# zhu-xlab/PFST

Measured on AMD Instinct MI355X. Metric: PFST train-step images/s on 1024² IRRG tiles, higher is better.
Workload: dtype f32 (f16x3 split MFMA: two scaled fp16 pieces per operand, three products, fp32 accumulate); 1 GPU; pfst_pots_irrg2vaih_irrg_deeplabv3plus_r50-d8; global_batch=8, per_gpu_batch=8, tile=1024x1024x3, num_classes=6, parallelism=dp1, weights=seeded random init, conv_math=f16x3

## Files before the change

### include/pfst_hip.h

```cpp
#ifndef PFST_HIP_H
#define PFST_HIP_H
#ifdef __cplusplus
extern "C" {
#endif

typedef void* pfst_stream_t;

int pfst_abi_version(void);
const char* pfst_last_error(void);
int pfst_set_deterministic(int on);
int pfst_get_deterministic(void);

int pfst_fill_f32(float* p, long long n, float value, pfst_stream_t stream);
int pfst_axpy_f32(float* y, const float* x, float alpha, long long n, pfst_stream_t stream);
int pfst_i64_to_u8(const long long* src, unsigned char* dst, long long n, pfst_stream_t stream);
int pfst_u8_to_i64(const unsigned char* src, long long* dst, long long n, pfst_stream_t stream);

typedef struct pfst_bnb_fuse {
  const float* x;
  long long x_bs;
  const float* y;
  long long y_bs;
  const float* coef;
  float* partials;
// ... 14 lines not shown
int pfst_conv_pack_weight_split(const float* w, void* wk6_fprop, void* wk6_dgrad, int Cout, int Cin, int T, pfst_stream_t stream);
int pfst_conv_igemm_split(const float* in, long long in_bs, const void* wk6, const float* bias, float* out, long long out_bs,
                          int N, int C, int Hi, int Wi, int M, int Ho, int Wo, int ksize, int stride, int dil, int pad,
                          int mode, int accumulate, float* stats, const pfst_bnb_fuse_t* bnb, pfst_stream_t stream);
int pfst_conv_wgrad_split(const float* x, long long x_bs, const float* dy, long long dy_bs, float* dw,
                          int N, int Cin, int Hi, int Wi, int Cout, int Ho, int Wo, int ksize, int stride, int dil, int pad,
                          pfst_stream_t stream);
int pfst_conv_wgrad(const float* x, long long x_bs, const float* dy, long long dy_bs, float* dw,
                    int N, int Cin, int Hi, int Wi, int Cout, int Ho, int Wo, int ksize, int stride, int dil, int pad,
                    pfst_stream_t stream);
int pfst_conv_wgrad_set_lds_pad(int bytes);
int pfst_bias_grad(const float* dy, long long dy_bs, float* db, int N, int C, int HW, pfst_stream_t stream);

int pfst_wino_tiles(int H, int W, int dil, int m);
int pfst_wino_pack_weight(const float* w, float* U_fprop, float* U_dgrad, int Cout, int Cin, int m, pfst_stream_t stream);
int pfst_wino_input(const float* x, long long x_bs, float* V, int N, int C, int H, int W, int dil, int m, float* v_amax,
                    const float* pack_x_amax, const float* bnl, pfst_stream_t stream);
int pfst_wino_gemm(const float* V, const float* U, float* Mbuf, int N, int K, int M, int T, int m, pfst_stream_t stream);
int pfst_wino_output(const float* Mbuf, float* y, long long y_bs, int N, int Cout, int H, int W, int dil, int accumulate,
                     float* stats, int stats_minmax, const float* bnb_x, long long bnb_x_bs, const float* bnb_coef, int bnb_relu, int m,
                     pfst_stream_t stream);
int pfst_wino_stats_slots(int H, int W, int dil, int m);
int pfst_wino_dy(const float* dy, long long dy_bs, float* dM, int N, int Cout, int H, int W, int dil, int m, float* dm_amax,
                 const float* pack_dy_amax, pfst_stream_t stream);
int pfst_wino_wgrad(const float* V, const float* dM, float* dU, float* dw, int N, int Cin, int Cout, int T, int m,
                    int split, const float* v_amax, const float* dm_amax, int packed, pfst_stream_t stream);
int pfst_wino_filter_plain(const float* w, float* P_fprop, float* P_dgrad, int Cout, int Cin, int m, pfst_stream_t stream);
int pfst_wino_pack_weight_split(const float* plain_f, const float* plain_d, void* U6_fprop, void* U6_dgrad, int Cout, int Cin,
                                int m, pfst_stream_t stream);
int pfst_wino_gemm_split(const float* V, const void* U6, float* Mbuf, int N, int K, int M, int T, int m, pfst_stream_t stream);

int pfst_absmax(const float* x, long long n, int planes, long long plane_stride, int slot_stride, float* slots, pfst_stream_t stream);
int pfst_conv_pack_weight_f16x2(const float* w, void* wk4_fprop, void* wk4_dgrad, int Cout, int Cin, int T, int sets,
                                const float* amax, pfst_stream_t stream);
typedef struct pfst_weight_job {
  const float* src;
  void* dst_f;
  void* dst_d;
  float* amax_f;
  float* amax_d;
  int Cout, Cin, T, sets, m, first_block;
} pfst_weight_job_t;
int pfst_weight_job_blocks(const pfst_weight_job_t* job, int pack);
int pfst_weight_prep_batched(const pfst_weight_job_t* jobs_host, const pfst_weight_job_t* jobs_dev, int njobs, pfst_stream_t stream);
int pfst_conv_pack_weight_f16x2_batched(const pfst_weight_job_t* jobs_host, const pfst_weight_job_t* jobs_dev, int njobs,
                                        pfst_stream_t stream);
int pfst_conv_igemm_f16x3(const float* in, long long in_bs, const void* wk4, const float* w_amax, const float* in_amax,
                          const float* bias, float* out, long long out_bs, int N, int C, int Hi, int Wi, int M, int Ho, int Wo,
                          int ksize, int stride, int dil, int pad, int mode, int accumulate, float* stats, const pfst_bnb_fuse_t* bnb,
                          const float* gate_dy, long long gate_dy_bs, const unsigned long long* gate_mask, int stats_minmax,
                          const float* bnl, pfst_stream_t stream);
int pfst_f16x3_set_slots(int slots);
int pfst_f16x3_chain_grid(long long total_tiles, int chainable);
int pfst_f16x3_split_probe(const float* x, long long n, const float* amax, unsigned* pieces_loop, unsigned* pieces_loop4,
                           unsigned* pieces_plain, pfst_stream_t stream);
int pfst_wino_gemm_f16x3(const float* V, const void* U4, const float* u_amax, const float* v_amax, float* Mbuf, int N, int K,
                         int M, int T, int m, int v_packed, pfst_stream_t stream);
int pfst_conv_wgrad_f16x3(const float* x, long long x_bs, const float* dy, long long dy_bs, float* dw, int N, int Cin, int Cout,
                          int HW, const float* x_amax, const float* dy_amax, const float* bnl, pfst_stream_t stream);
int pfst_conv_wgrad_f16x3_q(const float* x, long long x_bs, const float* dy, long long dy_bs, float* dw, int N, int Cin, int H, int W,
                            int Cout, int ksize, int dil, const float* x_amax, const float* dy_amax, pfst_stream_t stream);

int pfst_dwconv3x3(const float* x, long long x_bs, const float* w, float* y, long long y_bs,
                   int N, int C, int H, int W, int dil, int flip, int accumulate, float* stats, int stats_minmax,
                   const float* bn_on_load_coef, pfst_stream_t stream);
int pfst_dwconv_stats_slots(int H, int W, int dil);
int pfst_dwconv3x3_wgrad(const float* x, long long x_bs, const float* dy, long long dy_bs, float* dw,
                         int N, int C, int H, int W, int dil, pfst_stream_t stream);
int pfst_dwconv3x3_multi_ok(int H, int W, int ns, const int* dils);
int pfst_dwconv3x3_multi_fwd(const float* x, long long x_bs, int ns, const float* const* w, float* const* y, const long long* y_bs,
                             float* const* stats, int stats_minmax, const int* dils, float* plane_mean, int N, int C, int H, int W,
                             pfst_stream_t stream);
int pfst_dwconv3x3_multi_bwd(const float* x, long long x_bs, int ns, const float* const* w, const float* const* dy,
                             const long long* dy_bs, float* const* dw, const int* dils, const float* plane_mean_grad, float* dx,
                             long long dx_bs, int accumulate, const float* const* bn_pre, const pfst_bn_bwd_rec_t* const* bn_rec,
                             int N, int C, int H, int W, pfst_stream_t stream);
int pfst_dwconv3x3_bwd(const float* dy, long long dy_bs, const float* x, long long x_bs, const float* w, float* dx, long long dx_bs,
                       float* dw, int N, int C, int H, int W, int dil, int accumulate, const float* bn_on_load_coef,
                       const float* bn_pre, long long bn_pre_bs, const pfst_bn_bwd_rec_t* bn_rec, pfst_stream_t stream);

int pfst_bn_stats(const float* x, long long x_bs, int N, int C, int HW, float* mean, float* invstd,
                  float* running_mean, float* running_var, float momentum, float eps, double* ws,
                  const float* gamma, const float* beta, float* coef, pfst_stream_t stream);
int pfst_bn_finalize_partials(const float* partials, int T, int C, double count, float* mean, float* invstd,
                              float* running_mean, float* running_var, float momentum, float eps,
                              const float* gamma, const float* beta, float* coef, const float* minmax, int relu, float* y_amax,
                              pfst_stream_t stream);
int pfst_bn_apply(const float* x, long long x_bs, const float* residual, long long res_bs, float* y, long long y_bs,
                  const float* mean, const float* invstd, const float* gamma, const float* beta,
                  int N, int C, int HW, int relu, unsigned long long* relu_mask, float* y_amax, const float* post_scale,
                  const float* residual_coef, pfst_stream_t stream);
int pfst_bn_backward(const float* dy, long long dy_bs, const float* y, long long y_bs, const float* x, long long x_bs,
                     const float* mean, const float* invstd, const float* gamma, const float* beta,
                     float* dx, long long dx_bs, float* dres, long long dres_bs, int dres_accumulate,
                     float* dgamma, float* dbeta, int N, int C, int HW, int relu, const unsigned long long* relu_mask,
                     double* ws, const float* bwd_partials, int bwd_slots, float* dx_amax, const float* post_scale, pfst_stream_t stream);
int pfst_bn_backward_dual(const float* dy, long long dy_bs, const unsigned long long* relu_mask,
                          const float* xa, long long xa_bs, const float* mean_a, const float* invstd_a, const float* gamma_a,
                          float* dxa, long long dxa_bs, float* dgamma_a, float* dbeta_a, double* ws_a,
                          const float* bwd_partials_a, int bwd_slots_a, float* dxa_amax,
                          const float* xb, long long xb_bs, const float* mean_b, const float* invstd_b, const float* gamma_b,
                          float* dxb, long long dxb_bs, float* dgamma_b, float* dbeta_b, double* ws_b, float* dxb_amax,
                          int N, int C, int HW, pfst_stream_t stream);
int pfst_relu_gate(const float* g, long long g_bs, const unsigned long long* relu_mask, float* out, long long out_bs, int N, int C, int HW,
                   int accumulate, pfst_stream_t stream);
int pfst_bn_backward_sums(const float* dy, long long dy_bs, const float* x, long long x_bs, const float* mean, const float* invstd,
// ... 151 lines not shown
```

### pfst_amd/csrc/conv_f16x3.hip

```cpp
#include "conv_epilogue.h"
#include "amax.h"
#include "det.h"
#include "weight_jobs.h"
#include <math.h>
#include <stdlib.h>
#include <type_traits>
#include <utility>
#include "../../include/pfst_hip.h"

typedef _Float16 f16x8 __attribute__((ext_vector_type(8)));
typedef float f32x4 __attribute__((ext_vector_type(4)));

namespace {

constexpr int BN = 128;
constexpr int NP = 2;

template <int... Is, class F>
__device__ __forceinline__ void static_for_seq(std::integer_sequence<int, Is...>, F&& f) {
  (f(std::integral_constant<int, Is>()), ...);
}
template <int N, class F>
__device__ __forceinline__ void static_for(F&& f) {
  static_for_seq(std::make_integer_sequence<int, N>(), static_cast<F&&>(f));
// ... 445 lines not shown
                                                      reinterpret_cast<float*>(smem + PAIR_CHUNKS), gsrc, gmask, nullptr, nt_out);
          __syncthreads();
        } else
#endif
        conv_epilogue<TMW, 2, WAVES_N, BN>(acc32, outn, bias, stats, stats_T, accumulate, M, P, m0, p0, wm0, wn0, bx, n, wid, lane, PfstBnbArgs(), nullptr,
                                           gsrc, gmask, stats_mm, nt_out);
      }
#pragma unroll
      for (int i = 0; i < TMW; ++i)
#pragma unroll
        for (int j = 0; j < 2; ++j)
#pragma unroll
          for (int r = 0; r < 16; ++r) acc32[i][j][r] = 0.f;
    }
  };

  for (int lin = blockIdx.x; lin < total; lin += G) {
    if (!CHAIN || lin == (int)blockIdx.x) prologue(lin);
    for (int k = 0; k < KP; k += 2) {
      step32(std::integral_constant<int, 1>(), k);
      if (k + 1 < KP) step32(std::integral_constant<int, 0>(), k + 1);
    }
    epilogue(lin);
  }
}

template <int SHAPE, bool BPACK = false, bool ONE = false, int BMT = 128>
__global__ __launch_bounds__(BMT == 64 ? 256 : 2 * BMT, BMT == 256 ? 1 : 2) void conv_igemm_f16x3_kernel(
    const float* __restrict__ in, i64 in_bs, const uint4* __restrict__ wk4, const float* __restrict__ bias,
    float* __restrict__ out, i64 out_bs, int C, int Hi, int Wi, int M, int Ho, int Wo, int ks,
    int ca, int cb, int cc, int cdivv, int accumulate, float* __restrict__ stats, int stats_T,
    const float* __restrict__ w_amax, const float* __restrict__ in_amax, int Y, int Z, int chain, PfstResGate gate) {
  conv_igemm_f16x3_body<SHAPE, 0, BPACK, ONE, BMT>(in, in_bs, wk4, bias, out, out_bs, C, Hi, Wi, M, Ho, Wo, ks, ca, cb, cc, cdivv, accumulate, stats, stats_T,
                               w_amax, in_amax, Y, Z, chain, PfstBnbArgs(), gate);
}
__global__ __launch_bounds__(512, 1) void conv_igemm_f16x3_bnl_kernel(
    const float* __restrict__ in, i64 in_bs, const uint4* __restrict__ wk4, const float* __restrict__ bias,
    float* __restrict__ out, i64 out_bs, int C, int Hi, int Wi, int M, int Ho, int Wo, int ks,
    int ca, int cb, int cc, int cdivv, int accumulate, float* __restrict__ stats, int stats_T,
    const float* __restrict__ w_amax, const float* __restrict__ in_amax, int Y, int Z, int chain, const float4* __restrict__ bnl) {
  conv_igemm_f16x3_body<32, 0, false, true, 256, true>(in, in_bs, wk4, bias, out, out_bs, C, Hi, Wi, M, Ho, Wo, ks, ca, cb, cc, cdivv, accumulate, stats,
                                                       stats_T, w_amax, in_amax, Y, Z, chain, PfstBnbArgs(), PfstResGate(), bnl);
}
template <int BNB, bool ONE = false, int BMT = 128>
__global__ __launch_bounds__(2 * BMT, BMT == 128 ? 2 : 1) void conv_igemm_f16x3_bnb_kernel(
    const float* __restrict__ in, i64 in_bs, const uint4* __restrict__ wk4, const float* __restrict__ bias,
    float* __restrict__ out, i64 out_bs, int C, int Hi, int Wi, int M, int Ho, int Wo, int ks,
    int ca, int cb, int cc, int cdivv, int accumulate, float* __restrict__ stats, int stats_T,
    const float* __restrict__ w_amax, const float* __restrict__ in_amax, int Y, int Z, int chain, PfstBnbArgs bnb, PfstResGate gate) {
  conv_igemm_f16x3_body<32, BNB, false, ONE, BMT>(in, in_bs, wk4, bias, out, out_bs, C, Hi, Wi, M, Ho, Wo, ks, ca, cb, cc, cdivv, accumulate, stats, stats_T,
                                 w_amax, in_amax, Y, Z, chain, bnb, gate);
}


typedef float f32x16 __attribute__((ext_vector_type(16)));

struct Split4 {
  unsigned h[2], l[2];
  float t0[2], t1[2];
};
#ifdef PFST_F16X3_SPLIT6
template <int K>
__device__ __forceinline__ void split4_op_f16(const float (&v)[4], float s, Split4& st) {
  constexpr int q = K / 6, op = K % 6;
  if constexpr (op == 0) asm volatile("v_mul_f32 %0, %1, %2" : "=v"(st.t0[q]) : "s"(s), "v"(v[2 * q]));
  else if constexpr (op == 1) asm volatile("v_mul_f32 %0, %1, %2" : "=v"(st.t1[q]) : "s"(s), "v"(v[2 * q + 1]));
  else if constexpr (op == 2) asm volatile("v_cvt_pk_f16_f32 %0, %1, %2" : "=v"(st.h[q]) : "v"(st.t0[q]), "v"(st.t1[q]));
  else if constexpr (op == 3)
    asm volatile("v_fma_mix_f32 %0, %1, %2, -%3 op_sel:[0,0,0] op_sel_hi:[0,0,1]" : "=v"(st.t0[q]) : "v"(v[2 * q]), "s"(s), "v"(st.h[q]));
  else if constexpr (op == 4)
    asm volatile("v_fma_mix_f32 %0, %1, %2, -%3 op_sel:[0,0,1] op_sel_hi:[0,0,1]" : "=v"(st.t1[q]) : "v"(v[2 * q + 1]), "s"(s), "v"(st.h[q]));
  else asm volatile("v_cvt_pk_f16_f32 %0, %1, %2" : "=v"(st.l[q]) : "v"(st.t0[q]), "v"(st.t1[q]));
}
#else
template <int K>
__device__ __forceinline__ void split4_op_f16(const float (&v)[4], float s, Split4& st) {
  constexpr int q = K / 6, op = K % 6;
  if constexpr (op == 2) asm volatile("v_fma_mixlo_f16 %0, %1, %2, 0 op_sel_hi:[0,0,0]" : "=v"(st.h[q]) : "v"(v[2 * q]), "s"(s));
  else if constexpr (op == 3) asm volatile("v_fma_mixhi_f16 %0, %1, %2, 0 op_sel_hi:[0,0,0]" : "+v"(st.h[q]) : "v"(v[2 * q + 1]), "s"(s));
  else if constexpr (op == 4)
    asm volatile("v_fma_mixlo_f16 %0, %1, %2, -%3 op_sel:[0,0,0] op_sel_hi:[0,0,1]" : "=v"(st.l[q]) : "v"(v[2 * q]), "s"(s), "v"(st.h[q]));
  else if constexpr (op == 5)
    asm volatile("v_fma_mixhi_f16 %0, %1, %2, -%3 op_sel:[0,0,1] op_sel_hi:[0,0,1]" : "+v"(st.l[q]) : "v"(v[2 * q + 1]), "s"(s), "v"(st.h[q]));
}
#endif
template <int K>
__device__ __forceinline__ void unpack4_op_f16(const float (&v)[4], Split4& st) {
  constexpr int q = K & 1;
  if constexpr (K < 2) asm volatile("v_perm_b32 %0, %1, %2, %3" : "=v"(st.h[q]) : "v"(v[2 * q + 1]), "v"(v[2 * q]), "s"(0x05040100u));
  else asm volatile("v_perm_b32 %0, %1, %2, %3" : "=v"(st.l[q]) : "v"(v[2 * q + 1]), "v"(v[2 * q]), "s"(0x07060302u));
}

template <bool PACK, int BMT = 128, bool BNL = false>
__global__ __launch_bounds__(2 * BMT, BMT == 128 ? 2 : 1) void conv_wgrad_f16x3_line_kernel(
    const float* __restrict__ x, i64 x_bs, const float* __restrict__ dy, i64 dy_bs, float* __restrict__ dw,
    int J, int M, int P, int chunks, int chunk_len, int N, i64 x_gs, i64 dy_gs, i64 dw_gs, int gx, int gy, int gz,
    const float* __restrict__ x_amax, const float* __restrict__ dy_amax, const float4* __restrict__ bnl) {
  static_assert(!BNL || !PACK, "a pre-split operand is already normalised");
  constexpr int BM = BMT, BJ = 128, WM = 64, WAVES_N = 2, WN = 64, TM = 2, TN = 2, NT = 2 * BM;
  constexpr int RPP = NT / 8;
  constexpr int PA = BM / RPP, PB = BJ / RPP;
  constexpr int ROWS_A = BM + 2, ROWS_B = BJ + 2;
  constexpr int TILE_A = 4 * ROWS_A + 4, TILE_B = 4 * ROWS_B + 4;
  __shared__ uint4 As[2][2 * TILE_A];
  __shared__ uint4 Bs[2][2 * TILE_B];

// ... 109 lines not shown
      else if constexpr (e == 2) rd_b(t, 1, pb);
      else rd_a(t, 1, pa);
    };
    static_for<4>([&](auto rc) { read_frag(rc); });
    __builtin_amdgcn_sched_barrier(0);
    Split4 st[2];
    const int pk2 = pbeg + (kp + 2) * 32;
    static_for<24>([&](auto mc) {
      constexpr int m = decltype(mc)::value;
      constexpr int prod = m >> 3, t = (m >> 2) & 1, i = (m >> 1) & 1, j = m & 1;
      constexpr int pa = prod == 0 ? 1 : 0, pb = prod == 1 ? 1 : 0;
      acc[i][j] = __builtin_amdgcn_mfma_f32_32x32x16_f16(af[t][i][pa], bf[t][j][pb], acc[i][j], 0, 0, 0);
      if constexpr (m < 12) read_frag(std::integral_constant<int, 4 + m>());
      if constexpr (m < PA + PB) load_quad(mc, curc, pk2);
      constexpr int q = m / 3, part = m % 3;
      if constexpr (q < PA + PB) {
        constexpr int opb = q >= PA, pass = opb ? q - PA : q;
        if constexpr (BNL && opb && part == 0) normalise(lb[NXT][pass], pass);
        static_for<4>([&](auto kc) {
          constexpr int k = part * 4 + decltype(kc)::value;
          if constexpr (PACK) {
            if constexpr (k < 4) unpack4_op_f16<k>(opb ? lb[NXT][pass] : la[NXT][pass], st[q & 1]);
          } else {
            split4_op_f16<k>(opb ? lb[NXT][pass] : la[NXT][pass], opb ? sb : sa, st[q & 1]);
          }
        });
        if constexpr (part == 2) store_half(std::integral_constant<int, q>(), NXT, st[q & 1]);
      }
      __builtin_amdgcn_sched_barrier(0);
    });
    __syncthreads();
  };
  const int KPAIRS = (pend - pbeg + 31) / 32;
  for (int kp = 0; kp < KPAIRS; kp += 2) {
    step(std::integral_constant<int, 0>(), kp);
    if (kp + 1 < KPAIRS) step(std::integral_constant<int, 1>(), kp + 1);
  }
  const float ua = unscale_of(ea), ub = unscale_of(eb);
#pragma unroll
  for (int i = 0; i < TM; ++i) {
#pragma unroll
    for (int j = 0; j < TN; ++j) {
      const int jj = j0 + wn0 + j * 32 + l31;
#pragma unroll
      for (int r = 0; r < 16; ++r) {
        const int m = m0 + wm0 + i * 32 + (r & 3) + 8 * (r >> 2) + 4 * lh;
        if (m < M && jj < J) atomicAdd(&dw[(i64)m * J + jj], acc[i][j][r] * ua * ub);
      }
    }
  }
}

int f16x3_slots_override = 0;
unsigned f16x3_grid(i64 total, bool chainable, int wg_per_cu = 2) {
  static int cus = 0;
  if (cus == 0) {
    int dev = 0;
    if (hipGetDevice(&dev) != hipSuccess || hipDeviceGetAttribute(&cus, hipDeviceAttributeMultiprocessorCount, dev) != hipSuccess || cus <= 0) cus = 256;
  }
  int slots = (f16x3_slots_override > 0 ? f16x3_slots_override : 2 * cus) * wg_per_cu / 2;
  if (slots < 1) slots = 1;
  if (!chainable || total <= slots) return (unsigned)total;
  i64 best_g = total;
  double best_waste = 1e30;
  for (int t = 0; t <= 32; ++t) {
    const i64 g = t == 0 ? slots : (total + t - 1) / t;
    if (g < slots) continue;
    const i64 per_wg = (total + g - 1) / g, rounds = (g + slots - 1) / slots;
    if (per_wg > 8) continue;
    const double waste = (double)(rounds * per_wg * slots) / (double)total;
    if (waste < best_waste - 1e-9 || (waste < best_waste + 1e-9 && g < best_g)) { best_waste = waste; best_g = g; }
  }
  return (unsigned)best_g;
}


}

extern "C" int pfst_f16x3_set_slots(int slots) {
  PFST_CHECK_ARG(slots >= 0);
  f16x3_slots_override = slots;
  return PFST_OK;
}

extern "C" int pfst_f16x3_chain_grid(long long total_tiles, int chainable) {
  if (total_tiles <= 0 || total_tiles >= (1ll << 31)) return 0;
  return (int)f16x3_grid(total_tiles, chainable != 0);
}

namespace {
__global__ __launch_bounds__(256) void f16x3_split_probe_kernel(const float* __restrict__ x, i64 n8, const float* __restrict__ amax,
                                                                unsigned* __restrict__ pieces_loop, unsigned* __restrict__ pieces_loop4,
                                                                unsigned* __restrict__ pieces_plain) {
  const float s = __builtin_bit_cast(float, __builtin_amdgcn_readfirstlane(__builtin_bit_cast(int, scale_of(amax_exponent(amax_read(amax))))));
  for (i64 g = (i64)blockIdx.x * blockDim.x + threadIdx.x; g < n8; g += (i64)gridDim.x * blockDim.x) {
    float v[8];
#pragma unroll
    for (int j = 0; j < 8; ++j) v[j] = x[g * 8 + j];
    SplitF16 st;
    static_for<24>([&](auto kc) { split_op_f16<decltype(kc)::value>(v, s, st); });
    uint4 ph, pl;
    split8_f16(v, s, ph, pl);
    const unsigned hp[4] = {ph.x, ph.y, ph.z, ph.w}, lp[4] = {pl.x, pl.y, pl.z, pl.w};
#pragma unroll
    for (int q = 0; q < 4; ++q) {
      pieces_loop[g * 8 + 2 * q] = (st.h[q] & 0xffffu) | (st.l[q] << 16);
      pieces_loop[g * 8 + 2 * q + 1] = (st.h[q] >> 16) | (st.l[q] & 0xffff0000u);
      pieces_plain[g * 8 + 2 * q] = (hp[q] & 0xffffu) | (lp[q] << 16);
      pieces_plain[g * 8 + 2 * q + 1] = (hp[q] >> 16) | (lp[q] & 0xffff0000u);
    }
#pragma unroll
    for (int half = 0; half < 2; ++half) {
      const float v4[4] = {v[4 * half], v[4 * half + 1], v[4 * half + 2], v[4 * half + 3]};
      Split4 s4;
      static_for<12>([&](auto kc) { split4_op_f16<decltype(kc)::value>(v4, s, s4); });
#pragma unroll
      for (int q = 0; q < 2; ++q) {
        pieces_loop4[g * 8 + 4 * half + 2 * q] = (s4.h[q] & 0xffffu) | (s4.l[q] << 16);
        pieces_loop4[g * 8 + 4 * half + 2 * q + 1] = (s4.h[q] >> 16) | (s4.l[q] & 0xffff0000u);
      }
    }
  }
}
}

extern "C" int pfst_f16x3_split_probe(const float* x, long long n, const float* amax, unsigned* pieces_loop, unsigned* pieces_loop4,
                                      unsigned* pieces_plain, pfst_stream_t stream) {
  PFST_CHECK_ARG(x && amax && pieces_loop && pieces_loop4 && pieces_plain && n > 0 && n % 8 == 0);
  hipLaunchKernelGGL(f16x3_split_probe_kernel, dim3(ew_grid(n / 8)), dim3(256), 0, (hipStream_t)stream, x, (i64)(n / 8), amax, pieces_loop,
                     pieces_loop4, pieces_plain);
  PFST_CHECK_LAUNCH();
  return PFST_OK;
}

// ... 33 lines not shown
    PFST_CHECK_ARG(J.src && J.amax_f && (J.dst_f || J.dst_d) && J.Cout > 0 && J.Cin > 0 && (J.T == 1 || J.T == 9) && J.sets >= 1);
    PFST_CHECK_ARG((!J.dst_f || J.Cin % 16 == 0) && (!J.dst_d || J.Cout % 16 == 0) && (J.sets == 1 || J.T == 1) && J.first_block == blocks);
    blocks += weight_job_blocks(J, 1);
  }
  PFST_CHECK_ARG(blocks < (1ll << 31));
  hipLaunchKernelGGL(pack_weight_f16x2_batched_kernel, dim3((unsigned)blocks), dim3(256), 0, (hipStream_t)stream, jobs_dev, njobs);
  PFST_CHECK_LAUNCH();
  return PFST_OK;
}

extern "C" int pfst_conv_igemm_f16x3(const float* in, long long in_bs, const void* wk4, const float* w_amax, const float* in_amax,
                                     const float* bias, float* out, long long out_bs, int N, int C, int Hi, int Wi, int M, int Ho, int Wo,
                                     int ksize, int stride, int dil, int pad, int mode, int accumulate, float* stats,
                                     const pfst_bnb_fuse_t* bnb, const float* gate_dy, long long gate_dy_bs,
                                     const unsigned long long* gate_mask, int stats_minmax, const float* bnl, pfst_stream_t stream) {
  PFST_CHECK_ARG(in && wk4 && w_amax && in_amax && out && N > 0 && C > 0 && M > 0 && Hi > 0 && Wi > 0 && Ho > 0 && Wo > 0);
  PFST_CHECK_ARG(!bnl || (mode == 0 && ksize == 1 && stride == 1 && pad == 0 && M % 256 == 0 && C <= 2048 && !bias && !gate_dy && !(bnb && bnb->x) &&
                          !accumulate));
  PFST_CHECK_ARG(!stats_minmax || (stats && !bias && !(bnb && bnb->x)));
  PfstResGate gate;
  if (gate_dy) {
    PFST_CHECK_ARG(gate_mask && mode == 1 && !accumulate && !bias && !stats && M % 128 == 0 && ((i64)Ho * Wo) % 256 == 0 &&
                   gate_dy_bs >= (i64)M * Ho * Wo);
    gate.g = gate_dy;
    gate.g_bs = gate_dy_bs;
    gate.mask = gate_mask;
  }
  PFST_CHECK_ARG(!bnb || (bnb->x && bnb->x_bs >= (i64)M * Ho * Wo && (!bnb->y || bnb->y_bs >= (i64)M * Ho * Wo)));
  PFST_CHECK_ARG(!bnb || !bnb->y_mask || (bnb->y && bnb->relu && ((i64)Ho * Wo) % 256 == 0));
  PFST_CHECK_ARG((ksize == 1 || ksize == 3) && (stride == 1 || stride == 2) && dil >= 1 && pad >= 0 && (mode == 0 || mode == 1));
  PFST_CHECK_ARG(in_bs >= (i64)C * Hi * Wi && out_bs >= (i64)M * Ho * Wo && N <= 65535);
  PFST_CHECK_ARG((i64)C * Hi * Wi * 4 < (1ll << 31) && (i64)M * Ho * Wo * 4 < (1ll << 31) && (i64)ksize * ksize * C * M * 4 < (1ll << 31));
  if ((C % 32 != 0 && !(ksize == 1 && C % 16 == 0)) || M <= 32) {
    pfst_set_error(__FILE__, __LINE__, "f16x3 kernel needs C % 32 == 0 (1x1: C % 16 == 0) and more than 32 output channels (use pfst_conv_igemm_split)");
    return PFST_ERR_UNSUPPORTED;
  }
  const bool small = M <= 64;
  PFST_CHECK_ARG(!small || !(bnb && bnb->x));
  const int span = (ksize - 1) * dil;
  if (mode == 0) {
    PFST_CHECK_ARG(Ho == (Hi + 2 * pad - span - 1) / stride + 1 && Wo == (Wi + 2 * pad - span - 1) / stride + 1);
  } else {
    PFST_CHECK_ARG(Hi == (Ho + 2 * pad - span - 1) / stride + 1 && Wi == (Wo + 2 * pad - span - 1) / stride + 1);
  }
  int a, b, c, d;
  if (mode == 0) { a = stride; b = dil; c = -pad; d = 1; } else { a = 1; b = -dil; c = pad; d = stride; }
  const int stats_T = N * (int)cdiv((i64)Ho * Wo, BN) * 2;
  const bool one = !small && ksize == 1 && stride == 1 && pad == 0;
  const bool big = one && M % 256 == 0;
  const i64 total = (i64)cdiv((i64)Ho * Wo, BN) * cdiv(M, big ? 256 : small ? 64 : 128) * N;
  PFST_CHECK_ARG(total < (1ll << 31));
  const dim3 grid(f16x3_grid(total, one && ((C + 31) / 32) % 2 == 0, big ? 1 : 2));
  const int chain = 1 | (stats_minmax ? 2 : 0) | 4;
  if (bnb && bnb->x) {
    PFST_CHECK_ARG(M % 128 == 0 && !bias && !stats && bnb->coef && bnb->partials);
#define PFST_LAUNCH_F16_BNB(MODE_, ONE_)                                                                                                    \
    hipLaunchKernelGGL((conv_igemm_f16x3_bnb_kernel<MODE_, ONE_>), grid, dim3(256), 0, (hipStream_t)stream, in, (i64)in_bs, (const uint4*)wk4, bias, \
                       out, (i64)out_bs, C, Hi, Wi, M, Ho, Wo, ksize, a, b, c, d, accumulate, stats, stats_T, w_amax, in_amax, 1, N, chain, *bnb, gate)
#define PFST_LAUNCH_F16_BNB_BIG(MODE_)                                                                                                      \
    hipLaunchKernelGGL((conv_igemm_f16x3_bnb_kernel<MODE_, true, 256>), grid, dim3(512), 0, (hipStream_t)stream, in, (i64)in_bs, (const uint4*)wk4, bias, \
                       out, (i64)out_bs, C, Hi, Wi, M, Ho, Wo, ksize, a, b, c, d, accumulate, stats, stats_T, w_amax, in_amax, 1, N, chain, *bnb, gate)
    if (big) {
      if (!bnb->relu) PFST_LAUNCH_F16_BNB_BIG(3);
      else if (bnb->y_mask) PFST_LAUNCH_F16_BNB_BIG(4);
      else if (bnb->y) PFST_LAUNCH_F16_BNB_BIG(2);
      else PFST_LAUNCH_F16_BNB_BIG(1);
    } else if (one) {
      if (!bnb->relu) PFST_LAUNCH_F16_BNB(3, true);
      else if (bnb->y_mask) PFST_LAUNCH_F16_BNB(4, true);
      else if (bnb->y) PFST_LAUNCH_F16_BNB(2, true);
      else PFST_LAUNCH_F16_BNB(1, true);
    } else {
      if (!bnb->relu) PFST_LAUNCH_F16_BNB(3, false);
      else if (bnb->y_mask) PFST_LAUNCH_F16_BNB(4, false);
      else if (bnb->y) PFST_LAUNCH_F16_BNB(2, false);
      else PFST_LAUNCH_F16_BNB(1, false);
    }
#undef PFST_LAUNCH_F16_BNB
#undef PFST_LAUNCH_F16_BNB_BIG
    PFST_CHECK_LAUNCH();
    return PFST_OK;
  }
  if (bnl)
    hipLaunchKernelGGL(conv_igemm_f16x3_bnl_kernel, grid, dim3(512), 0, (hipStream_t)stream, in, (i64)in_bs, (const uint4*)wk4, bias, out, (i64)out_bs, C, Hi, Wi,
                       M, Ho, Wo, ksize, a, b, c, d, accumulate, stats, stats_T, w_amax, in_amax, 1, N, chain, reinterpret_cast<const float4*>(bnl));
  else if (small)
    hipLaunchKernelGGL((conv_igemm_f16x3_kernel<32, false, false, 64>), grid, dim3(256), 0, (hipStream_t)stream, in, (i64)in_bs, (const uint4*)wk4, bias, out,
                       (i64)out_bs, C, Hi, Wi, M, Ho, Wo, ksize, a, b, c, d, accumulate, stats, stats_T, w_amax, in_amax, 1, N, chain, gate);
  else if (big)
    hipLaunchKernelGGL((conv_igemm_f16x3_kernel<32, false, true, 256>), grid, dim3(512), 0, (hipStream_t)stream, in, (i64)in_bs, (const uint4*)wk4, bias, out,
                       (i64)out_bs, C, Hi, Wi, M, Ho, Wo, ksize, a, b, c, d, accumulate, stats, stats_T, w_amax, in_amax, 1, N, chain, gate);
  else if (one)
    hipLaunchKernelGGL((conv_igemm_f16x3_kernel<32, false, true>), grid, dim3(256), 0, (hipStream_t)stream, in, (i64)in_bs, (const uint4*)wk4, bias, out,
                       (i64)out_bs, C, Hi, Wi, M, Ho, Wo, ksize, a, b, c, d, accumulate, stats, stats_T, w_amax, in_amax, 1, N, chain, gate);
  else
    hipLaunchKernelGGL(conv_igemm_f16x3_kernel<32>, grid, dim3(256), 0, (hipStream_t)stream, in, (i64)in_bs, (const uint4*)wk4, bias, out,
                       (i64)out_bs, C, Hi, Wi, M, Ho, Wo, ksize, a, b, c, d, accumulate, stats, stats_T, w_amax, in_amax, 1, N, chain, gate);
  PFST_CHECK_LAUNCH();
  return PFST_OK;
}

extern "C" int pfst_wino_gemm_f16x3(const float* V, const void* U4, const float* u_amax, const float* v_amax, float* Mbuf, int N, int K,
                                    int M, int T, int m, int v_packed, pfst_stream_t stream) {
  PFST_CHECK_ARG(V && U4 && u_amax && v_amax && Mbuf && N > 0 && N <= 65535 && K > 0 && K % 32 == 0 && M > 64 && T > 0 && (m == 2 || m == 4));
  const int nx = (m + 2) * (m + 2);
  PFST_CHECK_ARG((i64)K * T * 4 < (1ll << 31) && (i64)M * T * 4 < (1ll << 31) && (i64)K * M * 4 < (1ll << 31));
  const bool big = M % 256 == 0;
  const i64 total = (i64)cdiv((i64)T, BN) * cdiv(M, big ? 256 : 128) * nx * N;
  PFST_CHECK_ARG(total < (1ll << 31));
  const dim3 grid(f16x3_grid(total, (K / 32) % 2 == 0, big ? 1 : 2));
  const int chain = 1 | 4;
  if (big && v_packed)
    hipLaunchKernelGGL((conv_igemm_f16x3_kernel<32, true, true, 256>), grid, dim3(512), 0, (hipStream_t)stream, V, (i64)K * T, (const uint4*)U4,
                       (const float*)nullptr, Mbuf, (i64)M * T, K, 1, T, M, 1, T, 1, 1, 1, 0, 1, 0, (float*)nullptr, 0, u_amax, v_amax, nx, N, chain, PfstResGate());
  else if (big)
    hipLaunchKernelGGL((conv_igemm_f16x3_kernel<32, false, true, 256>), grid, dim3(512), 0, (hipStream_t)stream, V, (i64)K * T, (const uint4*)U4,
                       (const float*)nullptr, Mbuf, (i64)M * T, K, 1, T, M, 1, T, 1, 1, 1, 0, 1, 0, (float*)nullptr, 0, u_amax, v_amax, nx, N, chain, PfstResGate());
  else if (v_packed)
    hipLaunchKernelGGL((conv_igemm_f16x3_kernel<32, true, true>), grid, dim3(256), 0, (hipStream_t)stream, V, (i64)K * T, (const uint4*)U4,
                       (const float*)nullptr, Mbuf, (i64)M * T, K, 1, T, M, 1, T, 1, 1, 1, 0, 1, 0, (float*)nullptr, 0, u_amax, v_amax, nx, N, chain, PfstResGate());
  else
    hipLaunchKernelGGL((conv_igemm_f16x3_kernel<32, false, true>), grid, dim3(256), 0, (hipStream_t)stream, V, (i64)K * T, (const uint4*)U4, (const float*)nullptr,
                       Mbuf, (i64)M * T, K, 1, T, M, 1, T, 1, 1, 1, 0, 1, 0, (float*)nullptr, 0, u_amax, v_amax, nx, N, chain, PfstResGate());
  PFST_CHECK_LAUNCH();
  return PFST_OK;
}

int pfst_wgrad_f16x3_launch(const float* x, i64 x_bs, const float* dy, i64 dy_bs, float* dw, int N, int J, int M, int P, int groups,
                            i64 x_gs, i64 dy_gs, i64 dw_gs, const float* x_amax, const float* dy_amax, int packed, hipStream_t s, const float* bnl) {
  PFST_CHECK_ARG(!bnl || (!packed && groups == 1));
  const float4* const bnl4 = reinterpret_cast<const float4*>(bnl);
  const bool big = M % 256 == 0;
  const int bm = big ? 256 : 128;
  const int tiles = cdiv(J, 128) * cdiv(M, bm) * groups;
  const double slots = big ? 256.0 : 256.0 * 2;
  int chunks = 1;
  double best = -1.0;
  for (int c = 1; c <= 64 && (c == 1 || P / c >= 512); ++c) {
    const double rounds = (double)tiles * N * c / slots;
// ... 41 lines not shown
```

### pfst_amd/hip_ops.py

```python
import ctypes
import os

import torch

from ._lib import call, lib

F32, U8, I64, F64 = torch.float32, torch.uint8, torch.int64, torch.float64


def _stream():
    return torch.cuda.current_stream().cuda_stream


def _chk(t, dtype=F32, nd=None):
    if not t.is_cuda:
        raise RuntimeError('pfst_amd ops run on the GPU only (got a CPU tensor); there is no CPU fallback')
    if t.dtype != dtype:
        raise TypeError(f'expected {dtype}, got {t.dtype}')
    if nd is not None and t.dim() != nd:
        raise ValueError(f'expected {nd}-d tensor, got shape {tuple(t.shape)}')
    return t


def _bs(t):
# ... 186 lines not shown

def conv_fprop(x, wk, cout, ksize, stride=1, dil=1, pad=0, bias=None, out=None, want_stats=False):
    return _conv_fprop('pfst_conv_igemm', 1, x, wk, cout, ksize, stride, dil, pad, bias, out, want_stats)


def conv_dgrad(dy, wk_d, cin, in_hw, ksize, stride=1, dil=1, pad=0, out=None, accumulate=False, bnb=None):
    return _conv_dgrad('pfst_conv_igemm', 1, dy, wk_d, cin, in_hw, ksize, stride, dil, pad, out, accumulate, bnb)


def pack_weight_split(w, want_fprop=True, want_dgrad=True, out_f=None, out_d=None):
    _dense(w)
    co, ci, kh, kw = w.shape
    wf, wd = _pack_outs(w, want_fprop, want_dgrad, out_f, out_d, (6 * co * ci * kh * kw,), dtype=U8)
    call('pfst_conv_pack_weight_split', w.data_ptr(), _p(wf), _p(wd), co, ci, kh * kw, _stream())
    return wf, wd


def conv_fprop_split(x, wk6, cout, ksize, stride=1, dil=1, pad=0, bias=None, out=None, want_stats=False):
    return _conv_fprop('pfst_conv_igemm_split', 6, x, wk6, cout, ksize, stride, dil, pad, bias, out, want_stats)


AMAX_SUB = 1024
_amax_arena = {}


def amax_slots(dev, groups=1):
    need = groups * AMAX_SUB
    key = (dev, torch.cuda.current_stream().cuda_stream)
    blk = _amax_arena.get(key)
    if blk is None or blk[1] + need > blk[0].numel():
        blk = [torch.zeros(max(1 << 22, need), dtype=F32, device=dev), 0]
        _amax_arena[key] = blk
    out = blk[0][blk[1]:blk[1] + need]
    blk[1] += need
    return out


def absmax(x, planes=1, out=None):
    if out is None:
        out = amax_slots(x.device, planes)
    if planes == 1 and x.dim() == 4 and not x.is_contiguous():
        n, c, h, w = x.shape
        call('pfst_absmax', x.data_ptr(), c * h * w, n, _bs(x), 0, out.data_ptr(), _stream())
        return out
    _dense(x)
    n = x.numel() // planes
    assert n * planes == x.numel()
    call('pfst_absmax', x.data_ptr(), n, planes, n, 1, out.data_ptr(), _stream())
    return out


def set_f16x3_slots(slots):
    call('pfst_f16x3_set_slots', int(slots))


def f16x3_eligible(cin, cout, ksize=3):
    return (cin % 32 == 0 or (ksize == 1 and cin % 16 == 0)) and cout > F16X3_MIN_ROWS


F16X3_MIN_ROWS = 32


def pack_weight_f16x2(w, want_fprop=True, want_dgrad=True, out_f=None, out_d=None, amax=None, sets=1):
    _dense(w)
    if sets == 1:
        co, ci, kh, kw = w.shape
        t = kh * kw
    else:
        assert w.dim() == 3 and w.shape[0] == sets
        _, co, ci = w.shape
        t = 1
    wf, wd = _pack_outs(w, want_fprop, want_dgrad, out_f, out_d, (4 * sets * co * ci * t,), dtype=U8)
    if amax is None:
        amax = absmax(w, sets)
    call('pfst_conv_pack_weight_f16x2', w.data_ptr(), _p(wf), _p(wd), co, ci, t, sets, amax.data_ptr(), _stream())
    return wf, wd, amax


class _WeightJob(ctypes.Structure):
    _fields_ = [('src', ctypes.c_void_p), ('dst_f', ctypes.c_void_p), ('dst_d', ctypes.c_void_p), ('amax_f', ctypes.c_void_p),
                ('amax_d', ctypes.c_void_p), ('Cout', ctypes.c_int), ('Cin', ctypes.c_int), ('T', ctypes.c_int), ('sets', ctypes.c_int),
                ('m', ctypes.c_int), ('first_block', ctypes.c_int)]


class WeightJobTable:

    def __init__(self, jobs, pack, dev):
        self.n = len(jobs)
        self.host = (_WeightJob * self.n)()
        first = 0
        for j, d in zip(self.host, jobs):
            j.src, j.dst_f, j.dst_d, j.amax_f, j.amax_d = (_p(d.get(k)) or None for k in ('src', 'dst_f', 'dst_d', 'amax_f', 'amax_d'))
            j.Cout, j.Cin, j.T, j.sets, j.m, j.first_block = d['Cout'], d['Cin'], d['T'], d.get('sets', 1), d.get('m', 0), first
            first += lib().pfst_weight_job_blocks(ctypes.addressof(j), pack)
        self.blocks = first
        self.dev = torch.frombuffer(bytearray(bytes(self.host)), dtype=U8).to(dev)
        self.keep = [t for d in jobs for t in d.values() if torch.is_tensor(t)]

    def run(self, name):
        call(name, ctypes.addressof(self.host), self.dev.data_ptr(), self.n, _stream())


BNL_MAX_C = 2048


def conv_fprop_bnl_ok(cin, cout, ksize, stride=1, pad=0):
# ... 1213 lines not shown
```

Before: 29.99 images/s.

## Add warp-specialized halo-tile kernel for small-channel 3x3 f16x3 convs

Adds a persistent 3x3 stride-1 conv kernel for 32/64-input-channel layers. Four producer waves load each output tile's input halo patch once, split it to fp16 hi/lo pieces into LDS, and prefetch the next tile. Four consumer waves run MFMA against that shared patch, replacing the per-tap gather and split of the generic small kernel. The cost is a large dynamic LDS allocation (one workgroup per CU), extra barriers between producer and consumers, and a new code path enabled by default for eligible layers.

After: 30.06 images/s, median of 6. About the same (+0.2%).

```diff
diff --git a/include/pfst_hip.h b/include/pfst_hip.h
--- a/include/pfst_hip.h
+++ b/include/pfst_hip.h
@@ -90,6 +90,7 @@
                           const float* bnl, pfst_stream_t stream);
 int pfst_f16x3_set_slots(int slots);
 int pfst_f16x3_chain_grid(long long total_tiles, int chainable);
+int pfst_f16x3_set_halo(int enabled);
 int pfst_f16x3_split_probe(const float* x, long long n, const float* amax, unsigned* pieces_loop, unsigned* pieces_loop4,
                            unsigned* pieces_plain, pfst_stream_t stream);
 int pfst_wino_gemm_f16x3(const float* V, const void* U4, const float* u_amax, const float* v_amax, float* Mbuf, int N, int K,
diff --git a/pfst_amd/csrc/conv_f16x3.hip b/pfst_amd/csrc/conv_f16x3.hip
--- a/pfst_amd/csrc/conv_f16x3.hip
+++ b/pfst_amd/csrc/conv_f16x3.hip
@@ -521,6 +521,182 @@
                                  w_amax, in_amax, Y, Z, chain, bnb, gate);
 }
 
+constexpr size_t HALO_LDS_MAX = 160 * 1024;
+constexpr int HALO_SLOTS = 2;
+__host__ __device__ __forceinline__ void halo_patch_geom(int p0, int P, int W, int& y0, int& cx0, int& pw, int& pr) {
+  const int p1 = (p0 + BN < P ? p0 + BN : P) - 1;
+  y0 = p0 / W;
+  const int y1 = p1 / W;
+  if (y0 == y1) {
+    cx0 = p0 - y0 * W - 1;
+    pw = p1 - p0 + 3;
+  } else {
+    cx0 = -1;
+    pw = W + 2;
+  }
+  pr = y1 - y0 + 3;
+}
+
+template <int SPT>
+__global__ __launch_bounds__(512, 1) void conv_igemm_f16x3_halo_kernel(
+    const float* __restrict__ in, i64 in_bs, const uint4* __restrict__ wk4, const float* __restrict__ bias, float* __restrict__ out, i64 out_bs,
+    int H, int W, int M, int tb, int tc, int accumulate, float* __restrict__ stats, int stats_T, const float* __restrict__ w_amax,
+    const float* __restrict__ in_amax, int Z, int chain) {
+  constexpr int C = 32 * SPT, CB8 = C / 8, KP = 9 * SPT, KT16 = (C / 16) * 9;
+  extern __shared__ uint4 halo_smem[];
+  uint4* const Ps = halo_smem;
+
+  const int tid = threadIdx.x, lane = tid & 63, wid = __builtin_amdgcn_readfirstlane(tid >> 6);
+  const int P = H * W;
+  const int gx = (P + BN - 1) / BN, total = gx * Z, G = gridDim.x;
+  constexpr unsigned OOB = 0x80000000u;
+  const int b_chan = P * 4;
+  const int eb = amax_exponent(amax_read(in_amax));
+  auto tile_of = [&](int lin, int& n, int& bx) {
+    n = lin / gx;
+    int by;
+    pfst_tile_order(lin - n * gx, gx, 1, 1, bx, by);
+  };
+
+  if (wid >= 4) {
+    const int lt = tid - 256;
+    const float sb = __builtin_bit_cast(float, __builtin_amdgcn_readfirstlane(__builtin_bit_cast(int, scale_of(eb))));
+    float raw[HALO_SLOTS][CB8][8];
+    auto issue = [&](int lin) {
+      int n, bx, y0, cx0, pw, pr;
+      tile_of(lin, n, bx);
+      halo_patch_geom(bx * BN, P, W, y0, cx0, pw, pr);
+      const int npx = pw * pr;
+      const __amdgpu_buffer_rsrc_t b_rsrc = __builtin_amdgcn_make_buffer_rsrc(const_cast<float*>(in) + (i64)n * in_bs, 0, C * P * 4, 0x00020000);
+#pragma unroll
+      for (int s = 0; s < HALO_SLOTS; ++s) {
+        if (__builtin_amdgcn_readfirstlane(lt & ~63) + 256 * s < npx) {
+          const int pp = lt + 256 * s;
+          const int r = pp / pw, c = pp - r * pw;
+          const int iy = y0 - 1 + r, ix = cx0 + c;
+          const unsigned voff = (pp < npx) & (iy >= 0) & (iy < H) & (ix >= 0) & (ix < W) ? 4u * (unsigned)(iy * W + ix) : OOB;
+#pragma unroll
+          for (int cb8 = 0; cb8 < CB8; ++cb8) {
+#pragma unroll
+            for (int i = 0; i < 8; ++i)
+              raw[s][cb8][i] = __builtin_bit_cast(float, __builtin_amdgcn_raw_buffer_load_b32(b_rsrc, voff, (cb8 * 8 + i) * b_chan, 0));
+          }
+        }
+      }
+    };
+    auto flush = [&](int lin) {
+      int n, bx, y0, cx0, pw, pr;
+      tile_of(lin, n, bx);
+      halo_patch_geom(bx * BN, P, W, y0, cx0, pw, pr);
+      const int npx = pw * pr;
+#pragma unroll
+      for (int s = 0; s < HALO_SLOTS; ++s) {
+        const int pp = lt + 256 * s;
+        if (pp < npx) {
+#pragma unroll
+          for (int cb8 = 0; cb8 < CB8; ++cb8) {
+            SplitF16 st;
+            static_for<24>([&](auto kc) { split_op_f16<decltype(kc)::value>(raw[s][cb8], sb, st); });
+            uint4* const dst = Ps + cb8 * NP * npx + pp;
+            dst[0] = make_uint4(st.h[0], st.h[1], st.h[2], st.h[3]);
+            dst[npx] = make_uint4(st.l[0], st.l[1], st.l[2], st.l[3]);
+          }
+        }
+      }
+    };
+#pragma unroll
+    for (int s = 0; s < HALO_SLOTS; ++s)
+#pragma unroll
+      for (int cb8 = 0; cb8 < CB8; ++cb8)
+#pragma unroll
+        for (int i = 0; i < 8; ++i) raw[s][cb8][i] = 0.f;
+    issue(blockIdx.x);
+    for (int lin = blockIdx.x; lin < total; lin += G) {
+      flush(lin);
+      __syncthreads();
+      if (lin + G < total) issue(lin + G);
+      __syncthreads();
+    }
+    return;
+  }
+
+  const int wm0 = (wid / 2) * 32, wn0 = (wid % 2) * 64;
+  const int l31 = lane & 31, lh = lane >> 5;
+  float* const stats_mm = (stats && (chain & 2)) ? stats + (i64)2 * M * stats_T : nullptr;
+  const bool nt_out = KP <= 16 && (chain & 4) != 0;
+  const int ea = amax_exponent(amax_read(w_amax));
+  const int a_chunk = 2 * M * 16;
+  const unsigned a_voff = wm0 + l31 < M ? 16u * ((unsigned)lh * (unsigned)M + (unsigned)(wm0 + l31)) : OOB;
+  const __amdgpu_buffer_rsrc_t a_rsrc = __builtin_amdgcn_make_buffer_rsrc(const_cast<uint4*>(wk4), 0, KT16 * 2 * NP * M * 16, 0x00020000);
+  pfst_f32x16 acc32[1][2];
+#pragma unroll
+  for (int j = 0; j < 2; ++j)
+#pragma unroll
+    for (int r = 0; r < 16; ++r) acc32[0][j][r] = 0.f;
+
+  for (int lin = blockIdx.x; lin < total; lin += G) {
+    int n, bx, y0, cx0, pw, pr;
+    tile_of(lin, n, bx);
+    const int p0 = bx * BN;
+    halo_patch_geom(p0, P, W, y0, cx0, pw, pr);
+    const int npx = pw * pr;
+    constexpr int AHEAD = 2;
+    f16x8 af[AHEAD + 1][2][NP];
+    f16x8 bf[2][2][2][NP];
+    auto load_a = [&](auto kc) {
+      constexpr int k = decltype(kc)::value;
+#pragma unroll
+      for (int t = 0; t < 2; ++t)
+#pragma unroll
+        for (int pl = 0; pl < NP; ++pl)
+          af[k % (AHEAD + 1)][t][pl] = __builtin_bit_cast(f16x8, __builtin_amdgcn_raw_buffer_load_b128(a_rsrc, a_voff, ((2 * k + t) * NP + pl) * a_chunk, 0));
+    };
+    static_for<AHEAD>([&](auto kc) { load_a(kc); });
+    int lb[2];
+#pragma unroll
+    for (int j = 0; j < 2; ++j) {
+      const int p = p0 + wn0 + j * 32 + l31;
+      const int oy = p / W, ox = p - oy * W;
+      lb[j] = (p < P ? (oy - y0) * pw + (ox - cx0) : 1) + lh * NP * npx;
+    }
+    auto read_b = [&](auto kc) {
+      constexpr int k = decltype(kc)::value, tap = k / SPT, cb = k % SPT, ty = tap / 3, tx = tap % 3;
+      const int so = cb * 4 * NP * npx + (ty * tb + tc + 1) * pw + (tx * tb + tc);
+#pragma unroll
+      for (int t = 0; t < 2; ++t)
+#pragma unroll
+        for (int j = 0; j < 2; ++j)
+#pragma unroll
+          for (int pl = 0; pl < NP; ++pl) bf[k % 2][t][j][pl] = __builtin_bit_cast(f16x8, Ps[lb[j] + so + (t * 2 * NP + pl) * npx]);
+    };
+    __syncthreads();
+    read_b(std::integral_constant<int, 0>());
+    static_for<KP>([&](auto kc) {
+      constexpr int k = decltype(kc)::value;
+      if constexpr (k + AHEAD < KP) load_a(std::integral_constant<int, k + AHEAD>());
+      if constexpr (k + 1 < KP) read_b(std::integral_constant<int, k + 1>());
+      static_for<12>([&](auto mc) {
+        constexpr int m = decltype(mc)::value;
+        constexpr int prod = m / 4, rem = m % 4, t = rem / 2, j = rem & 1;
+        constexpr int pa = prod == 0 ? 1 : 0, pb = prod == 1 ? 1 : 0;
+        acc32[0][j] = __builtin_amdgcn_mfma_f32_32x32x16_f16(af[k % (AHEAD + 1)][t][pa], bf[k % 2][t][j][pb], acc32[0][j], 0, 0, 0);
+      });
+    });
+    __syncthreads();
+
+    const float ua = unscale_of(ea), ub = unscale_of(eb);
+#pragma unroll
+    for (int j = 0; j < 2; ++j)
+#pragma unroll
+      for (int r = 0; r < 16; ++r) acc32[0][j][r] = acc32[0][j][r] * ua * ub;
+    conv_epilogue<1, 2, 2, BN>(acc32, out + (i64)n * out_bs, bias, stats, stats_T, accumulate, M, P, 0, p0, wm0, wn0, bx, n, wid, lane, PfstBnbArgs(), nullptr,
+                               nullptr, nullptr, stats_mm, nt_out);
+#pragma unroll
+    for (int j = 0; j < 2; ++j)
+#pragma unroll
+      for (int r = 0; r < 16; ++r) acc32[0][j][r] = 0.f;
+  }
+}
 
 typedef float f32x16 __attribute__((ext_vector_type(16)));
 
@@ -736,6 +912,25 @@
 }
 
 int f16x3_slots_override = 0;
+int f16x3_halo_enabled = 1;
+
+size_t f16x3_halo_lds(int C, int H, int W) {
+  if (C != 32 && C != 64) return 0;
+  const int P = H * W;
+  int npx = 0;
+  if (W % BN == 0) {
+    npx = 3 * (BN + 2);
+  } else {
+    for (int p0 = 0; p0 < P; p0 += BN) {
+      int y0, cx0, pw, pr;
+      halo_patch_geom(p0, P, W, y0, cx0, pw, pr);
+      if (pw * pr > npx) npx = pw * pr;
+    }
+  }
+  const size_t bytes = (size_t)(C / 8) * NP * npx * sizeof(uint4);
+  return npx <= 256 * HALO_SLOTS && bytes <= HALO_LDS_MAX ? bytes : 0;
+}
+
 unsigned f16x3_grid(i64 total, bool chainable, int wg_per_cu = 2) {
   static int cus = 0;
   if (cus == 0) {
@@ -764,6 +959,12 @@
 extern "C" int pfst_f16x3_set_slots(int slots) {
   PFST_CHECK_ARG(slots >= 0);
   f16x3_slots_override = slots;
+  return PFST_OK;
+}
+
+extern "C" int pfst_f16x3_set_halo(int enabled) {
+  PFST_CHECK_ARG(enabled == 0 || enabled == 1);
+  f16x3_halo_enabled = enabled;
   return PFST_OK;
 }
 
@@ -903,6 +1104,7 @@
   PFST_CHECK_ARG(total < (1ll << 31));
   const dim3 grid(f16x3_grid(total, one && ((C + 31) / 32) % 2 == 0, big ? 1 : 2));
   const int chain = 1 | (stats_minmax ? 2 : 0) | 4;
+  const size_t halo_lds = (small && f16x3_halo_enabled && ksize == 3 && stride == 1 && dil == 1 && pad == 1 && !gate_dy && !bnl) ? f16x3_halo_lds(C, Hi, Wi) : 0;
   if (bnb && bnb->x) {
     PFST_CHECK_ARG(M % 128 == 0 && !bias && !stats && bnb->coef && bnb->partials);
 #define PFST_LAUNCH_F16_BNB(MODE_, ONE_)                                                                                                    \
@@ -935,7 +1137,29 @@
   if (bnl)
     hipLaunchKernelGGL(conv_igemm_f16x3_bnl_kernel, grid, dim3(512), 0, (hipStream_t)stream, in, (i64)in_bs, (const uint4*)wk4, bias, out, (i64)out_bs, C, Hi, Wi,
                        M, Ho, Wo, ksize, a, b, c, d, accumulate, stats, stats_T, w_amax, in_amax, 1, N, chain, reinterpret_cast<const float4*>(bnl));
-  else if (small)
+  else if (halo_lds) {
+    int dev = 0, cus = 0;
+    if (hipGetDevice(&dev) != hipSuccess || hipDeviceGetAttribute(&cus, hipDeviceAttributeMultiprocessorCount, dev) != hipSuccess || cus <= 0) cus = 256;
+    const dim3 hgrid((unsigned)(total < cus ? total : cus));
+    static bool lds_set_on[64] = {};
+    bool& lds_set = lds_set_on[dev & 63];
+    if (!lds_set) {
+      hipError_t e = hipFuncSetAttribute(reinterpret_cast<const void*>(&conv_igemm_f16x3_halo_kernel<1>), hipFuncAttributeMaxDynamicSharedMemorySize, (int)HALO_LDS_MAX);
+      if (e == hipSuccess)
+        e = hipFuncSetAttribute(reinterpret_cast<const void*>(&conv_igemm_f16x3_halo_kernel<2>), hipFuncAttributeMaxDynamicSharedMemorySize, (int)HALO_LDS_MAX);
+      if (e != hipSuccess) {
+        pfst_set_error(__FILE__, __LINE__, hipGetErrorString(e));
+        return PFST_ERR_LAUNCH;
+      }
+      lds_set = true;
+    }
+#define PFST_LAUNCH_HALO(SPT_)                                                                                                              \
+    hipLaunchKernelGGL(conv_igemm_f16x3_halo_kernel<SPT_>, hgrid, dim3(512), halo_lds, (hipStream_t)stream, in, (i64)in_bs, (const uint4*)wk4, bias, out, \
+                       (i64)out_bs, Hi, Wi, M, b, c, accumulate, stats, stats_T, w_amax, in_amax, N, chain)
+    if (C == 32) PFST_LAUNCH_HALO(1);
+    else PFST_LAUNCH_HALO(2);
+#undef PFST_LAUNCH_HALO
+  } else if (small)
     hipLaunchKernelGGL((conv_igemm_f16x3_kernel<32, false, false, 64>), grid, dim3(256), 0, (hipStream_t)stream, in, (i64)in_bs, (const uint4*)wk4, bias, out,
                        (i64)out_bs, C, Hi, Wi, M, Ho, Wo, ksize, a, b, c, d, accumulate, stats, stats_T, w_amax, in_amax, 1, N, chain, gate);
   else if (big)
diff --git a/pfst_amd/hip_ops.py b/pfst_amd/hip_ops.py
--- a/pfst_amd/hip_ops.py
+++ b/pfst_amd/hip_ops.py
@@ -262,6 +262,10 @@
 
 def set_f16x3_slots(slots):
     call('pfst_f16x3_set_slots', int(slots))
+
+
+def set_f16x3_halo(enabled):
+    call('pfst_f16x3_set_halo', int(bool(enabled)))
 
 
 def f16x3_eligible(cin, cout, ksize=3):
```
